# retab-dev/k-LLMs

Measured on NVIDIA H100. Metric: consensus records/sec at n=16 (1M x 32-field); achieved HBM GB/s vs peak, higher is better.
Workload: dtype i32 codes / f64 values

## Files before the change

k_llms_b200/csrc/kc_numeric.cuh:

```cuda
#pragma once

#include <type_traits>
#include <utility>

#include "kc_common.cuh"
#include "kc_csa.cuh"
#include "kc_vote.cuh"

namespace kc {

constexpr uint32_t kNoneHi = (uint32_t)(KC_F64_NONE_BITS >> 32);
constexpr uint32_t kAbsentHi = (uint32_t)(KC_F64_ABSENT_BITS >> 32);
constexpr uint32_t kKeyNonFinite = 0xFFE00000u;

__device__ __forceinline__ int ffs_m(uint32_t m) { return __ffs((int)m); }
__device__ __forceinline__ int ffs_m(uint64_t m) { return __ffsll((long long)m); }
__device__ __forceinline__ int clz_m(uint32_t m) { return __clz((int)m); }
__device__ __forceinline__ int clz_m(uint64_t m) { return __clzll((long long)m); }

__device__ __constant__ double kPow10[13] = {1e-6, 1e-5, 1e-4, 1e-3, 1e-2, 1e-1, 1.0, 1e1, 1e2, 1e3, 1e4, 1e5, 1e6};


__device__ __forceinline__ double lds_f64(uint32_t addr) {
    double v;
    asm volatile("ld.shared.f64 %0, [%1];" : "=d"(v) : "r"(addr));
    return v;
}
__device__ __forceinline__ void sts_f64(uint32_t addr, double v) {
    asm volatile("st.shared.f64 [%0], %1;" ::"r"(addr), "d"(v) : "memory");
}
__device__ __forceinline__ uint2 lds_u32x2(uint32_t addr) {
    uint2 v;
    asm volatile("ld.shared.v2.u32 {%0,%1}, [%2];" : "=r"(v.x), "=r"(v.y) : "r"(addr));
    return v;
}

struct PlaneRow {
    uint32_t base, pitch;
    __device__ __forceinline__ uint32_t addr(uint32_t elem) const { return base + elem * pitch; }
    __device__ __forceinline__ uint32_t addr_mad(uint32_t elem) const {
        uint32_t a;
        asm("mad.lo.u32 %0, %1, %2, %3;" : "=r"(a) : "r"(elem), "r"(pitch), "r"(base));
        return a;
    }
};


template <typename F>
__device__ __forceinline__ double np_sum(F f, int n) {
    double res;
    if (n < 8) {
        res = -0.0;
        for (int i = 0; i < n; ++i) res = __dadd_rn(res, f(i));
    } else {
        double r0 = f(0), r1 = f(1), r2 = f(2), r3 = f(3), r4 = f(4), r5 = f(5), r6 = f(6), r7 = f(7);
        int i = 8;
        const int n8 = n - (n & 7);
        for (; i < n8; i += 8) {
            r0 = __dadd_rn(r0, f(i + 0));
            r1 = __dadd_rn(r1, f(i + 1));
            r2 = __dadd_rn(r2, f(i + 2));
            r3 = __dadd_rn(r3, f(i + 3));
            r4 = __dadd_rn(r4, f(i + 4));
            r5 = __dadd_rn(r5, f(i + 5));
            r6 = __dadd_rn(r6, f(i + 6));
            r7 = __dadd_rn(r7, f(i + 7));
        }
        res = __dadd_rn(__dadd_rn(__dadd_rn(r0, r1), __dadd_rn(r2, r3)), __dadd_rn(__dadd_rn(r4, r5), __dadd_rn(r6, r7)));
        for (; i < n; ++i) res = __dadd_rn(res, f(i));
    }
    return __dadd_rn(0.0, res);
}

template <typename Row>
__device__ __forceinline__ double np_mean(const Row &xs, int s, int len) {
    return __ddiv_rn(np_sum([&](int i) { return lds_f64(xs.addr(s + i)); }, len), (double)len);
}

template <typename Row>
__device__ __forceinline__ double np_mean16(const Row &xs, int s, int len) {
    const uint32_t a0 = xs.addr_mad((uint32_t)s);
    const uint32_t pitch = xs.addr(1) - xs.addr(0);
    double res;
    if (len < 8) {
        res = -0.0;
#pragma unroll
        for (int j = 0; j < 7; ++j)
            if (j < len) res = __dadd_rn(res, lds_f64(a0 + j * pitch));
    } else {
        double r[8];
#pragma unroll
        for (int j = 0; j < 8; ++j) r[j] = lds_f64(a0 + j * pitch);
        int tail = 8;
        if (len >= 16) {
#pragma unroll
            for (int j = 0; j < 8; ++j) r[j] = __dadd_rn(r[j], lds_f64(a0 + (8 + j) * pitch));
            tail = 16;
        }
        res = __dadd_rn(__dadd_rn(__dadd_rn(r[0], r[1]), __dadd_rn(r[2], r[3])),
                        __dadd_rn(__dadd_rn(r[4], r[5]), __dadd_rn(r[6], r[7])));
#pragma unroll
        for (int j = 0; j < 7; ++j)
            if (tail + j < len) res = __dadd_rn(res, lds_f64(a0 + (tail + j) * pitch));
    }
    return __ddiv_rn(__dadd_rn(0.0, res), (double)len);
}

template <typename Row>
__device__ __forceinline__ double np_median(const Row &xs, int s, int len) {
    if (len & 1) return __dadd_rn(0.0, __dadd_rn(-0.0, lds_f64(xs.addr(s + len / 2))));
    return __ddiv_rn(
        __dadd_rn(0.0, __dadd_rn(__dadd_rn(-0.0, lds_f64(xs.addr(s + len / 2 - 1))), lds_f64(xs.addr(s + len / 2)))), 2.0);
}

template <typename Row>
__device__ __forceinline__ double np_std(const Row &xs, int s, int len) {
    const double mean = np_mean(xs, s, len);
    const double ss = np_sum(
        [&](int i) {
            const double d = __dadd_rn(lds_f64(xs.addr(s + i)), -mean);
            return __dmul_rn(d, d);
        },
        len);
    return __dsqrt_rn(__ddiv_rn(ss, (double)len));
}

__device__ __forceinline__ double dmax(double a, double b) { return a > b ? a : b; }

__device__ __forceinline__ bool is_close(double a, double b, double rel_eps, double abs_eps) {
    const double denom = dmax(dmax(fabs(a), fabs(b)), 1.0);
    return fabs(__dadd_rn(a, -b)) <= dmax(abs_eps, __dmul_rn(rel_eps, denom));
}

__device__ __forceinline__ bool is_close_pow10(double a, double b, double rel_eps, double abs_eps) {
    if (a == 0.0 || b == 0.0) return is_close(a, b, rel_eps, abs_eps);
    for (int k = 0; k < 13; ++k)
        if (is_close(a, __dmul_rn(b, kPow10[k]), rel_eps, abs_eps)) return true;
    return false;
}

struct TieResult {
    double value;
    int support;
};

template <typename M, typename Row>
__device__ __noinline__ TieResult numeric_tie(const Row xs, M starts, int m, int top, double rel_eps, double abs_eps) {
    int best_s = -1, best_support = 0;
    double best_spread = 0.0, best_center = 0.0;
    M sk = starts;
    while (sk) {
        const int s = ffs_m(sk) - 1;
        sk &= sk - 1;
        const int e = sk ? ffs_m(sk) - 1 : m;
        const int len = e - s;
        if (len != top) continue;
        const double center = np_median(xs, s, len);
        int support = top;
        M so = starts;
        while (so) {
            const int os = ffs_m(so) - 1;
            so &= so - 1;
            const int oe = so ? ffs_m(so) - 1 : m;
            const int olen = oe - os;
            if (olen >= top) continue;
            const double oc = np_median(xs, os, olen);
            if (is_close(center, oc, rel_eps, abs_eps) || is_close(fabs(center), fabs(oc), rel_eps, abs_eps) ||
                is_close_pow10(center, oc, rel_eps, abs_eps))
                support += olen;
        }
        const double spread = len > 1 ? np_std(xs, s, len) : 0.0;
        const bool better = best_s < 0 || support > best_support ||
                            (support == best_support &&
                             (spread < best_spread || (spread == best_spread && fabs(center) > fabs(best_center))));
        if (better) {
            best_s = s;
            best_support = support;
            best_spread = spread;
            best_center = center;
        }
    }
    return TieResult{np_mean(xs, best_s, top), best_support};
}


template <int N>
struct BatcherNet {
    int a[N * N / 2 + 1];
    int b[N * N / 2 + 1];
    int count;
    constexpr BatcherNet() : a{}, b{}, count(0) {
        for (int p = 1; p < N; p *= 2)
            for (int k = p; k >= 1; k /= 2)
                for (int j = k % p; j <= N - 1 - k; j += 2 * k)
                    for (int i = 0; i < k; ++i)
                        if (i + j + k < N && (i + j) / (2 * p) == (i + j + k) / (2 * p)) {
                            a[count] = i + j;
                            b[count] = i + j + k;
                            ++count;
                        }
    }
};

template <int A, int B, int N>
__device__ __forceinline__ void compare_exchange(uint32_t (&x)[N]) {
    const uint32_t lo = min(x[A], x[B]), hi = max(x[A], x[B]);
    x[A] = lo;
    x[B] = hi;
}

template <int N, size_t... I>
__device__ __forceinline__ void sort_keys_impl(uint32_t (&x)[N], std::index_sequence<I...>) {
    constexpr BatcherNet<N> net{};
    (compare_exchange<net.a[I], net.b[I], N>(x), ...);
}

template <int N>
__device__ __forceinline__ void sort_keys(uint32_t (&x)[N]) {
    constexpr BatcherNet<N> net{};
    sort_keys_impl<N>(x, std::make_index_sequence<net.count>{});
}

__device__ __forceinline__ uint32_t far_bit(double d, double p, double q, double thr, uint32_t bit) {
    uint32_t r;
    asm("{\n\t"
        ".reg .pred c;\n\t"
        "setp.le.f64 c, %1, %2;\n\t"
        "setp.le.or.f64 c, %1, %3, c;\n\t"
        "setp.le.or.f64 c, %1, %4, c;\n\t"
        "selp.u32 %0, 0, %5, c;\n\t"
        "}"
        : "=r"(r)
        : "d"(d), "d"(p), "d"(q), "d"(thr), "r"(bit));
    return r;
}

template <typename Row>
__device__ __noinline__ void repair_sorted_prefix(const Row row, int m) {
    for (int i = 1; i < m; ++i) {
        const double v = lds_f64(row.addr(i));
        int j = i - 1;
        while (j >= 0) {
            const double u = lds_f64(row.addr(j));
            if (!(u > v)) break;
            sts_f64(row.addr(j + 1), u);
            --j;
        }
        sts_f64(row.addr(j + 1), v);
    }
}


template <int N, typename Row>
__device__ __forceinline__ void numeric_core(const uint32_t (&hi)[N], const Row row, double rel_eps, double abs_eps,
                                             double thr, double &value, uint32_t &meta) {
    using M = typename MaskOf<N>::type;
    static_assert(N >= 2 && (N & (N - 1)) == 0, "N must be a power of two >= 2");
    constexpr uint32_t IDX = N - 1;
    const double qnan = __longlong_as_double(0x7FF8000000000000LL);

    constexpr uint32_t Z_NONE = ((kNoneHi ^ 0x80000000u) - 0x00100000u) - kKeyNonFinite;
    static_assert(kAbsentHi == kNoneHi + 1, "tags must be adjacent high words");
    uint32_t key[N];
    uint32_t census = 0;
#pragma unroll
    for (int i = 0; i < N; ++i) {
        const uint32_t s = (uint32_t)((int32_t)hi[i] >> 31);
        const uint32_t t = (hi[i] ^ (s | 0x80000000u)) - 0x00100000u;
        key[i] = (t | IDX) - (IDX - (uint32_t)i);
        const uint32_t z = t - kKeyNonFinite;
        const uint32_t u = z - Z_NONE;
        const uint32_t tagged_inc = (u < 2u) ? (u + 0x10100u) : 0x100u;
        census += (z < 0x00200000u) ? tagged_inc : 0u;
    }
    const int m = N - (int)((census >> 8) & 0xFFu);
    const int present = N - (int)(census & 0xFFu);
    const int nn = N - (int)(census >> 16);
    if (nn == 0) {
        value = qnan;
        meta = pack_meta(0, 0, 0, present, 0);
        return;
    }
    if (nn == 1) {
        int idx = 0;
        for (int i = 0; i < N; ++i) {
            const uint32_t h = lds_u32x2(row.addr(i)).y;
            if (h != kNoneHi && h != kAbsentHi) idx = i;
        }
        value = lds_f64(row.addr(idx));
        meta = pack_meta(idx, 1, 1, present, KC_FLAG_HAS_VALUE | KC_FLAG_SINGLE);
        return;
    }
    if (m == 0) {
        value = qnan;
        meta = pack_meta(0, 0, nn, present, KC_FLAG_NO_FINITE);
        return;
    }

    sort_keys<N>(key);
    double xs[N];
#pragma unroll
    for (int k = 0; k < N; ++k) xs[k] = lds_f64(row.addr_mad(key[k] & IDX));

    bool unsorted = false;
#pragma unroll
    for (int k = 1; k < N; ++k) unsorted |= xs[k] < xs[k - 1];
#pragma unroll
    for (int k = 0; k < N; ++k) sts_f64(row.addr(k), xs[k]);
    if (unsorted) {
        repair_sorted_prefix<Row>(row, m);
#pragma unroll
        for (int k = 0; k < N; ++k) xs[k] = lds_f64(row.addr(k));
    }

    M starts = 1;
    {
        double p_prev = __dmul_rn(rel_eps, xs[0]);
#pragma unroll
        for (int k = 1; k < N; ++k) {
            const double p = __dmul_rn(rel_eps, xs[k]);
            const double d = __dadd_rn(xs[k], -xs[k - 1]);
            starts |= (M)far_bit(d, p, -p_prev, thr, 1u << (k & 31)) << (k & 32);
            p_prev = p;
        }
    }
    if (m < N) starts &= (M(1) << m) - 1;

    int top = 0, n_top = 0, top_s = 0;
    {
        const int c = m >> 1;
        const M below = starts & ((M(2) << c) - 1);
        const int s0 = (int)(sizeof(M) * 8 - 1) - clz_m(below);
        const M above = c + 1 < (int)(sizeof(M) * 8) ? (starts >> (c + 1)) : M(0);
        const int e0 = above ? c + ffs_m(above) : m;
        if (2 * (e0 - s0) > m) {
            top = e0 - s0;
            n_top = 1;
            top_s = s0;
        }
    }
    if (n_top == 0) {
        M sk = starts;
        while (sk) {
            const int s = ffs_m(sk) - 1;
            sk &= sk - 1;
            const int e = sk ? ffs_m(sk) - 1 : m;
            const int len = e - s;
            if (len > top) {
                top = len;
                n_top = 1;
                top_s = s;
            } else if (len == top) {
                ++n_top;
            }
        }
    }
    uint32_t flags = KC_FLAG_HAS_VALUE;
    int support = top;
    if (n_top == 1) {
        if constexpr (N <= 16 && std::is_same<Row, PlaneRow>::value)
            value = np_mean16(row, top_s, top);
        else
            value = np_mean(row, top_s, top);
    } else {
        const TieResult tr = numeric_tie<M, Row>(row, starts, m, top, rel_eps, abs_eps);
        value = tr.value;
        support = tr.support;
        flags |= KC_FLAG_TIE;
    }
    meta = pack_meta(0, support, nn, present, flags);
}

__device__ __forceinline__ void numeric_pair(uint2 a, uint2 b, double rel_eps, double abs_eps, double &value, uint32_t &meta) {
    const bool a_abs = a.y == kAbsentHi, b_abs = b.y == kAbsentHi;
    const bool a_nn = !a_abs && a.y != kNoneHi, b_nn = !b_abs && b.y != kNoneHi;
    const bool a_fin = a_nn && (a.y & 0x7FF00000u) != 0x7FF00000u, b_fin = b_nn && (b.y & 0x7FF00000u) != 0x7FF00000u;
    const uint32_t present = (a_abs ? 0u : 1u) + (b_abs ? 0u : 1u), nn = (a_nn ? 1u : 0u) + (b_nn ? 1u : 0u);
    const double va = __hiloint2double((int)a.y, (int)a.x), vb = __hiloint2double((int)b.y, (int)b.x);
    const double qnan = __longlong_as_double(0x7FF8000000000000ll);
    if (nn == 0) {
        value = qnan;
        meta = pack_meta(0, 0, 0, present, 0);
    } else if (nn == 1) {
        value = a_nn ? va : vb;
        meta = pack_meta(a_nn ? 0u : 1u, 1, 1, present, KC_FLAG_HAS_VALUE | KC_FLAG_SINGLE);
    } else if (!a_fin && !b_fin) {
        value = qnan;
        meta = pack_meta(0, 0, 2, present, KC_FLAG_NO_FINITE);
    } else if (a_fin != b_fin) {
        value = __dadd_rn(0.0, __dadd_rn(-0.0, a_fin ? va : vb));
        meta = pack_meta(0, 1, 2, present, KC_FLAG_HAS_VALUE);
    } else {
        const bool swap = va > vb;
        const double lo = swap ? vb : va, hi = swap ? va : vb;
        if (is_close(lo, hi, rel_eps, abs_eps)) {
            value = __ddiv_rn(__dadd_rn(0.0, __dadd_rn(__dadd_rn(-0.0, lo), hi)), 2.0);
            meta = pack_meta(0, 2, 2, present, KC_FLAG_HAS_VALUE);
        } else {
            const double c_lo = __dadd_rn(0.0, __dadd_rn(-0.0, lo)), c_hi = __dadd_rn(0.0, __dadd_rn(-0.0, hi));
            value = fabs(c_hi) > fabs(c_lo) ? c_hi : c_lo;
            meta = pack_meta(0, 1, 2, present, KC_FLAG_HAS_VALUE | KC_FLAG_TIE);
        }
    }
}

__global__ void __launch_bounds__(256) numeric_pairs_kernel(const double *__restrict__ vals, int64_t n_units, double rel_eps, double abs_eps,
                                                            double *__restrict__ out_value, uint32_t *__restrict__ out_meta) {
    const int64_t stride = (int64_t)gridDim.x * blockDim.x;
    int64_t u = (int64_t)blockIdx.x * blockDim.x + threadIdx.x;
    int4 cur[4];
    if (u < n_units) {
        const int4 *p = reinterpret_cast<const int4 *>(vals) + u * 4;
#pragma unroll
        for (int q = 0; q < 4; ++q) cur[q] = ldg_nc_v4(p + q);
    }
    for (; u < n_units; u += stride) {
        int4 nxt[4];
        if (u + stride < n_units) {
            const int4 *p = reinterpret_cast<const int4 *>(vals) + (u + stride) * 4;
#pragma unroll
            for (int q = 0; q < 4; ++q) nxt[q] = ldg_nc_v4(p + q);
        }
        double v[4];
        uint32_t m[4];
#pragma unroll
        for (int q = 0; q < 4; ++q)
            numeric_pair(make_uint2((uint32_t)cur[q].x, (uint32_t)cur[q].y), make_uint2((uint32_t)cur[q].z, (uint32_t)cur[q].w), rel_eps, abs_eps,
                         v[q], m[q]);
        double *ov = out_value + u * 4;
        asm volatile("st.global.L1::no_allocate.v2.f64 [%0], {%1,%2};" ::"l"(ov), "d"(v[0]), "d"(v[1]) : "memory");
        asm volatile("st.global.L1::no_allocate.v2.f64 [%0], {%1,%2};" ::"l"(ov + 2), "d"(v[2]), "d"(v[3]) : "memory");
        asm volatile("st.global.L1::no_allocate.v4.u32 [%0], {%1,%2,%3,%4};" ::"l"(out_meta + u * 4), "r"(m[0]), "r"(m[1]), "r"(m[2]), "r"(m[3])
                     : "memory");
#pragma unroll
        for (int q = 0; q < 4; ++q) cur[q] = nxt[q];
    }
}

__device__ __forceinline__ void cex(double &a, double &b) {
    const bool sw = a > b;
    const double lo = sw ? b : a, hi = sw ? a : b;
    a = lo;
    b = hi;
}

__device__ __forceinline__ void numeric_quad(const uint2 (&w)[4], double rel_eps, double abs_eps, double &value, uint32_t &meta) {
    const double pinf = __longlong_as_double(0x7FF0000000000000ll), qnan = __longlong_as_double(0x7FF8000000000000ll);
    uint32_t present = 0, nn = 0, m = 0, first_nn = 0;
    double x[4];
#pragma unroll
    for (int i = 3; i >= 0; --i) {
        const bool absent = w[i].y == kAbsentHi, none = w[i].y == kNoneHi, fin = (w[i].y & 0x7FF00000u) != 0x7FF00000u;
        present += absent ? 0u : 1u;
        const bool is_nn = !absent && !none;
        nn += is_nn ? 1u : 0u;
        first_nn = is_nn ? (uint32_t)i : first_nn;
        m += fin ? 1u : 0u;
        x[i] = fin ? __hiloint2double((int)w[i].y, (int)w[i].x) : pinf;
    }
    if (nn == 0) {
        value = qnan;
        meta = pack_meta(0, 0, 0, present, 0);
        return;
    }
    if (nn == 1) {
        const uint2 c = first_nn == 0 ? w[0] : (first_nn == 1 ? w[1] : (first_nn == 2 ? w[2] : w[3]));
        value = __hiloint2double((int)c.y, (int)c.x);
        meta = pack_meta(first_nn, 1, 1, present, KC_FLAG_HAS_VALUE | KC_FLAG_SINGLE);
        return;
    }
    if (m == 0) {
        value = qnan;
        meta = pack_meta(0, 0, nn, present, KC_FLAG_NO_FINITE);
        return;
    }
    cex(x[0], x[1]);
    cex(x[2], x[3]);
    cex(x[0], x[2]);
    cex(x[1], x[3]);
    cex(x[1], x[2]);
    const bool b0 = m > 1 && is_close(x[0], x[1], rel_eps, abs_eps);
    const bool b1 = m > 2 && is_close(x[1], x[2], rel_eps, abs_eps);
    const bool b2 = m > 3 && is_close(x[2], x[3], rel_eps, abs_eps);
    uint32_t best_len = 0, best_start = 0, n_top = 0, cur_len = 0, cur_start = 0;
#pragma unroll
    for (int i = 0; i < 4; ++i) {
        const bool in = (uint32_t)i < m;
        const bool joins = i > 0 && (i == 1 ? b0 : (i == 2 ? b1 : b2));
        cur_start = joins ? cur_start : (uint32_t)i;
        cur_len = joins ? cur_len + 1u : 1u;
        const bool ends = in && ((uint32_t)i + 1u == m || !(i == 0 ? b0 : (i == 1 ? b1 : b2)));
        if (ends) {
            if (cur_len > best_len) {
                best_len = cur_len;
                best_start = cur_start;
                n_top = 1;
            } else if (cur_len == best_len) {
                ++n_top;
            }
        }
    }
    auto mean_of = [&](uint32_t s, uint32_t z) -> double {
        double acc = -0.0;
#pragma unroll
        for (int i = 0; i < 4; ++i)
            if ((uint32_t)i >= s && (uint32_t)i < s + z) acc = __dadd_rn(acc, x[i]);
        return __ddiv_rn(__dadd_rn(0.0, acc), (double)z);
    };
    if (n_top == 1) {
        value = mean_of(best_start, best_len);
        meta = pack_meta(0, best_len, nn, present, KC_FLAG_HAS_VALUE);
        return;
    }
    if (best_len == 1) {
        double best = __dadd_rn(0.0, __dadd_rn(-0.0, x[0]));
#pragma unroll
        for (int i = 1; i < 4; ++i) {
            const double c = __dadd_rn(0.0, __dadd_rn(-0.0, x[i]));
            if ((uint32_t)i < m && fabs(c) > fabs(best)) best = c;
        }
        value = best;
        meta = pack_meta(0, 1, nn, present, KC_FLAG_HAS_VALUE | KC_FLAG_TIE);
        return;
    }
    auto pair_stats = [&](double a, double b, double &mean, double &sd) {
        mean = __ddiv_rn(__dadd_rn(0.0, __dadd_rn(__dadd_rn(-0.0, a), b)), 2.0);
        const double ta = __dadd_rn(a, -mean), tb = __dadd_rn(b, -mean);
        const double ss = __dadd_rn(0.0, __dadd_rn(__dadd_rn(-0.0, __dmul_rn(ta, ta)), __dmul_rn(tb, tb)));
        sd = __dsqrt_rn(__ddiv_rn(ss, 2.0));
    };
    double ma, sa, mb, sb;
    pair_stats(x[0], x[1], ma, sa);
    pair_stats(x[2], x[3], mb, sb);
    const bool second = sb < sa || (sb == sa && fabs(mb) > fabs(ma));
    value = second ? mb : ma;
    meta = pack_meta(0, 2, nn, present, KC_FLAG_HAS_VALUE | KC_FLAG_TIE);
}

__global__ void __launch_bounds__(256) numeric_quads_kernel(const double *__restrict__ vals, int64_t n_units, double rel_eps, double abs_eps,
                                                            double *__restrict__ out_value, uint32_t *__restrict__ out_meta) {
    const int64_t stride = (int64_t)gridDim.x * blockDim.x;
    int64_t u = (int64_t)blockIdx.x * blockDim.x + threadIdx.x;
    int4 cur[4];
    if (u < n_units) {
        const int4 *p = reinterpret_cast<const int4 *>(vals) + u * 4;
#pragma unroll
        for (int q = 0; q < 4; ++q) cur[q] = ldg_nc_v4(p + q);
    }
    for (; u < n_units; u += stride) {
        int4 nxt[4];
        if (u + stride < n_units) {
            const int4 *p = reinterpret_cast<const int4 *>(vals) + (u + stride) * 4;
#pragma unroll
            for (int q = 0; q < 4; ++q) nxt[q] = ldg_nc_v4(p + q);
        }
        double v[2];
        uint32_t m[2];
#pragma unroll
        for (int g = 0; g < 2; ++g) {
            const uint2 w[4] = {make_uint2((uint32_t)cur[2 * g].x, (uint32_t)cur[2 * g].y), make_uint2((uint32_t)cur[2 * g].z, (uint32_t)cur[2 * g].w),
                                make_uint2((uint32_t)cur[2 * g + 1].x, (uint32_t)cur[2 * g + 1].y),
                                make_uint2((uint32_t)cur[2 * g + 1].z, (uint32_t)cur[2 * g + 1].w)};
            numeric_quad(w, rel_eps, abs_eps, v[g], m[g]);
        }
        asm volatile("st.global.L1::no_allocate.v2.f64 [%0], {%1,%2};" ::"l"(out_value + u * 2), "d"(v[0]), "d"(v[1]) : "memory");
        asm volatile("st.global.L1::no_allocate.v2.u32 [%0], {%1,%2};" ::"l"(out_meta + u * 2), "r"(m[0]), "r"(m[1]) : "memory");
#pragma unroll
        for (int q = 0; q < 4; ++q) cur[q] = nxt[q];
    }
}



template <int NP, int T, bool PREFETCH>
__global__ void __launch_bounds__(T) numeric_direct_kernel(const double *__restrict__ vals, int64_t n_groups, int n,
                                                           double rel_eps, double abs_eps, double *__restrict__ out_value,
                                                           uint32_t *__restrict__ out_meta, const __grid_constant__ OutRoute mc) {
    extern __shared__ __align__(1024) uint8_t smem_raw[];
    const PlaneRow row{smem_u32(smem_raw) + threadIdx.x * 8u, T * 8u};
    const double thr = abs_eps > rel_eps ? abs_eps : rel_eps;
    const int64_t stride = (int64_t)gridDim.x * T;
    int64_t g = (int64_t)blockIdx.x * T + threadIdx.x;
    int4 cur[NP / 2 > 0 ? NP / 2 : 1];
    if constexpr (PREFETCH) {
        if (g < n_groups) {
            const int4 *p4 = reinterpret_cast<const int4 *>(vals + g * NP);
#pragma unroll
            for (int q = 0; q < NP / 2; ++q) cur[q] = ldg_nc_v4(p4 + q);
        }
    }
    for (; g < n_groups; g += stride) {
        uint32_t hi[NP];
        if constexpr (PREFETCH) {
            int4 nxt[NP / 2];
            if (g + stride < n_groups) {
                const int4 *p4 = reinterpret_cast<const int4 *>(vals + (g + stride) * NP);
#pragma unroll
                for (int q = 0; q < NP / 2; ++q) nxt[q] = ldg_nc_v4(p4 + q);
            }
#pragma unroll
            for (int q = 0; q < NP / 2; ++q) {
                hi[2 * q + 0] = (uint32_t)cur[q].y;
                hi[2 * q + 1] = (uint32_t)cur[q].w;
                sts_f64(row.addr(2 * q + 0), __hiloint2double(cur[q].y, cur[q].x));
                sts_f64(row.addr(2 * q + 1), __hiloint2double(cur[q].w, cur[q].z));
            }
            double v;
            uint32_t m;
            numeric_core<NP, PlaneRow>(hi, row, rel_eps, abs_eps, thr, v, m);
            store_out_f64(out_value + g, v, mc);
            store_out_u32(out_meta + g, m, mc);
#pragma unroll
            for (int q = 0; q < NP / 2; ++q) cur[q] = nxt[q];
        } else {
            const double *p = vals + g * n;
            if (n == NP) {
                const int4 *p4 = reinterpret_cast<const int4 *>(p);
#pragma unroll
                for (int q = 0; q < NP / 2; ++q) {
                    const int4 t = ldg_nc_v4(p4 + q);
                    hi[2 * q + 0] = (uint32_t)t.y;
                    hi[2 * q + 1] = (uint32_t)t.w;
                    sts_f64(row.addr(2 * q + 0), __hiloint2double(t.y, t.x));
                    sts_f64(row.addr(2 * q + 1), __hiloint2double(t.w, t.z));
                }
            } else {
#pragma unroll
                for (int i = 0; i < NP; ++i) {
                    const double v = (i < n) ? __ldg(p + i) : __longlong_as_double((long long)KC_F64_ABSENT_BITS);
                    hi[i] = (uint32_t)__double2hiint(v);
                    sts_f64(row.addr(i), v);
                }
            }
            double v;
            uint32_t m;
            numeric_core<NP, PlaneRow>(hi, row, rel_eps, abs_eps, thr, v, m);
            store_out_f64(out_value + g, v, mc);
            store_out_u32(out_meta + g, m, mc);
        }
    }
}


__device__ __forceinline__ void count_equal(uint32_t x, uint32_t key, uint32_t &n) {
    asm("{\n\t.reg .pred p;\n\t"
        "setp.eq.u32 p, %1, %2;\n\t"
        "@p add.u32 %0, %0, 1;\n\t}"
        : "+r"(n)
        : "r"(x), "r"(key));
}

__device__ __forceinline__ void match_cell(uint32_t h, uint32_t l, uint32_t hv, uint32_t lv, uint32_t &c, uint32_t &bad) {
    asm("{\n\t.reg .pred p;\n\t"
        "setp.eq.u32 p, %2, %4;\n\t"
        "@p add.u32 %0, %0, 1;\n\t"
        "@p lop3.b32 %1, %1, %3, %5, 0xF6;\n\t}"
        : "+r"(c), "+r"(bad)
        : "r"(h), "r"(l), "r"(hv), "r"(lv));
}

constexpr uint32_t kFastBias = 0x00100000u;

struct FastDecision {
    double v;
    uint32_t c, tagged, absent;
};

template <int N>
__device__ __forceinline__ bool numeric_fast_decide(const uint32_t (&x)[N], const uint32_t (&lo)[N], uint32_t top, double rel_eps,
                                                    double thr, FastDecision &out) {
    constexpr uint32_t X_NONE = kNoneHi + kFastBias, X_ABSENT = kAbsentHi + kFastBias;
    constexpr int PLANES = 32 - __builtin_clz((unsigned)N);
    uint32_t plane[PLANES];
    bit_counts(x, plane);
    const uint32_t xv = plane[PLANES - 1] | plane[PLANES - 2], lv = at_least_half(lo);
    uint32_t nonfinite = 0;
#pragma unroll
    for (int k = 0; k < PLANES; ++k) nonfinite += (plane[k] >> 31) << k;
    uint32_t c = 0, bad = 0, below = 0, above = 0xFFFFFFFFu, low_nf = 0xFFFFFFFFu, absent = 0;
    const uint32_t neg_xv = 0u - xv, neg_xv1 = ~xv;
#pragma unroll
    for (int i = 0; i < N; ++i) {
        below = max(below, x[i] + neg_xv);
        above = min(above, x[i] + neg_xv1);
        low_nf = min(low_nf, x[i] + 0x80000000u);
        match_cell(x[i], lo[i], xv, lv, c, bad);
    }
    if (top == kAbsentHi) {
#pragma unroll
        for (int i = 0; i < N; ++i) count_equal(x[i], X_ABSENT, absent);
    }
    const uint32_t tagged = nonfinite;
    if (top > kAbsentHi || (xv & 0x80000000u) != 0 || bad != 0 || 2 * c + nonfinite <= (uint32_t)N || tagged > (uint32_t)(N - 2) ||
        (nonfinite != 0 && low_nf < X_NONE - 0x80000000u))
        return false;
    const uint32_t hv = xv - kFastBias;
    const double v = __hiloint2double((int)hv, (int)lv);
    const uint32_t hb = hv + below, ha = hv + above + 1u;
    const double db = __dadd_rn(v, -__hiloint2double((int)hb, -1));
    const double da = __dadd_rn(__hiloint2double((int)ha, 0), -v);
    const bool far_b = db > thr && db > __dmul_rn(rel_eps, v);
    const bool far_a = da > thr && da > __dmul_rn(rel_eps, __hiloint2double((int)ha, -1));
    const bool has_b = below >= 0x80000000u, has_a = above < 0x7FFFFFFFu && ha < 0x7FF00000u;
    if ((has_b && !far_b) || (has_a && !far_a)) return false;
    out.v = v;
    out.c = c;
    out.tagged = tagged;
    out.absent = absent;
    return true;
}

template <int N>
__device__ __forceinline__ void numeric_fast_finish(const FastDecision &d, double &value, uint32_t &meta) {
    const double v = d.v;
    const uint32_t c = d.c, tagged = d.tagged, absent = d.absent;
    double res = -0.0;
    if (c >= 8) {
        double r = v;
#pragma unroll
        for (int k = 2; k <= N / 8; ++k)
            if ((int)(c >> 3) >= k) r = __dadd_rn(r, v);
        res = __dmul_rn(r, 8.0);
    }
    const uint32_t tail = c & 7u;
#pragma unroll
    for (int k = 1; k <= 7; ++k)
        if ((int)tail >= k) res = __dadd_rn(res, v);
    value = __ddiv_rn(__dadd_rn(0.0, res), (double)c);
    meta = (c << 6) + (((uint32_t)N - tagged) << 13) + (((uint32_t)N - absent) << 20) + ((uint32_t)KC_FLAG_HAS_VALUE << 27);
}

template <int NP, int T>
__global__ void __launch_bounds__(T) numeric_direct_fast_kernel(const double *__restrict__ vals, int64_t n_groups, double rel_eps,
                                                                double abs_eps, double *__restrict__ out_value,
                                                                uint32_t *__restrict__ out_meta, const __grid_constant__ OutRoute ) {
    extern __shared__ __align__(1024) uint8_t smem_raw[];
    __shared__ int64_t defer_q[T / 32][64];
    const PlaneRow row{smem_u32(smem_raw) + threadIdx.x * 8u, T * 8u};
    const double thr = abs_eps > rel_eps ? abs_eps : rel_eps;
    const int lane = threadIdx.x & 31;
    int64_t *my_q = defer_q[threadIdx.x >> 5];
    int q_count = 0;
    const int64_t stride = (int64_t)gridDim.x * T;
    const int64_t g0 = (int64_t)blockIdx.x * T + threadIdx.x;

    const uint32_t warp_plane = smem_u32(smem_raw) + (threadIdx.x & ~31u) * 8u;
    auto drain = [&](int count) {
        if (lane < count) {
            const int64_t g = my_q[lane];
            uint32_t hi[NP];
#pragma unroll
            for (int i = 0; i < NP; ++i) hi[i] = lds_u32x2(row.addr(i)).y;
            double v;
            uint32_t m;
            numeric_core<NP, PlaneRow>(hi, row, rel_eps, abs_eps, thr, v, m);
            store_local_f64(out_value + g, v);
            store_local_u32(out_meta + g, m);
        }
        __syncwarp();
    };

    int4 cur[NP / 2];
    if (g0 < n_groups) {
        const int4 *p4 = reinterpret_cast<const int4 *>(vals + g0 * NP);
#pragma unroll
        for (int q = 0; q < NP / 2; ++q) cur[q] = ldg_nc_v4(p4 + q);
    }
    for (int64_t gw = g0 - lane; gw < n_groups; gw += stride) {
        const int64_t g = gw + lane;
        int4 nxt[NP / 2];
        if (g + stride < n_groups) {
            const int4 *p4 = reinterpret_cast<const int4 *>(vals + (g + stride) * NP);
#pragma unroll
            for (int q = 0; q < NP / 2; ++q) nxt[q] = ldg_nc_v4(p4 + q);
        }
        uint32_t x[NP], lo[NP], top = 0;
#pragma unroll
        for (int q = 0; q < NP / 2; ++q) {
            lo[2 * q + 0] = (uint32_t)cur[q].x;
            x[2 * q + 0] = (uint32_t)cur[q].y + kFastBias;
            lo[2 * q + 1] = (uint32_t)cur[q].z;
            x[2 * q + 1] = (uint32_t)cur[q].w + kFastBias;
            top = max(top, max((uint32_t)cur[q].y, (uint32_t)cur[q].w));
        }
        FastDecision fd;
        const bool decided = numeric_fast_decide<NP>(x, lo, top, rel_eps, thr, fd);
        const bool defer = !decided && g < n_groups;
        const uint32_t dm = __ballot_sync(0xFFFFFFFFu, defer);
        if (defer) {
            const uint32_t slot = (uint32_t)q_count + (uint32_t)__popc(dm & ((1u << lane) - 1u));
            my_q[slot] = g;
            if (slot < 32u) {
#pragma unroll
                for (int i = 0; i < NP; ++i)
                    sts_f64(warp_plane + slot * 8u + (uint32_t)i * (T * 8u), __hiloint2double((int)(x[i] - kFastBias), (int)lo[i]));
            }
        }
        q_count += __popc(dm);
        if (decided && g < n_groups) {
            double v;
            uint32_t m;
            numeric_fast_finish<NP>(fd, v, m);
            store_local_f64(out_value + g, v);
            store_local_u32(out_meta + g, m);
        }
        __syncwarp();
        if (q_count >= 32) {
            drain(32);
            q_count -= 32;
            const int64_t moved = (lane < q_count) ? my_q[32 + lane] : 0;
            __syncwarp();
            if (lane < q_count) {
                my_q[lane] = moved;
                const int4 *p4 = reinterpret_cast<const int4 *>(vals + moved * NP);
#pragma unroll
                for (int q = 0; q < NP / 2; ++q) {
                    const int4 v4 = ldg_nc_v4(p4 + q);
                    sts_f64(row.addr(2 * q + 0), __hiloint2double(v4.y, v4.x));
                    sts_f64(row.addr(2 * q + 1), __hiloint2double(v4.w, v4.z));
                }
            }
            __syncwarp();
        }
#pragma unroll
        for (int q = 0; q < NP / 2; ++q) cur[q] = nxt[q];
    }
    if (q_count > 0) drain(q_count);
}

template <int N, int WARPS, int STAGES, int MIN_CTAS>
__global__ void __launch_bounds__(WARPS * 32, MIN_CTAS) numeric_tma_fast_kernel(const __grid_constant__ CUtensorMap tmap,
                                                                      const double *__restrict__ in, int64_t n_groups,
                                                                      double rel_eps, double abs_eps,
                                                                      double *__restrict__ out_value,
                                                                      uint32_t *__restrict__ out_meta, const __grid_constant__ OutRoute ) {
    constexpr int ROW_BYTES = N * 8;
    constexpr int BOX_ROWS_PER_GROUP = ROW_BYTES > 128 ? ROW_BYTES / 128 : 1;
    constexpr uint32_t TILE_BYTES = 32 * ROW_BYTES;
    constexpr int T = WARPS * 32;
    static_assert(TILE_BYTES % 1024 == 0, "warp tile must keep the swizzle atom alignment");
    extern __shared__ __align__(1024) uint8_t smem_raw[];
    uint8_t *smem = reinterpret_cast<uint8_t *>((reinterpret_cast<uintptr_t>(smem_raw) + 1023) & ~uintptr_t(1023));
    __shared__ __align__(8) uint64_t full_bar[WARPS * STAGES];
    __shared__ int64_t defer_q[WARPS][64];

    const int lane = threadIdx.x & 31;
    const int warp = threadIdx.x >> 5;
    uint8_t *my_smem = smem + (size_t)warp * STAGES * TILE_BYTES;
    uint64_t *my_bar = full_bar + warp * STAGES;
    int64_t *my_q = defer_q[warp];
    int q_count = 0;
    const PlaneRow row{smem_u32(smem + (size_t)WARPS * STAGES * TILE_BYTES) + threadIdx.x * 8u, T * 8u};
    const double thr = abs_eps > rel_eps ? abs_eps : rel_eps;

    const int64_t n_tiles = (n_groups + 31) >> 5;
    const int64_t first = (int64_t)blockIdx.x * WARPS + warp;
    const int64_t step = (int64_t)gridDim.x * WARPS;
    uint64_t policy = 0;

    if (lane == 0) {
        tma_prefetch_desc(&tmap);
#pragma unroll
        for (int s = 0; s < STAGES; ++s) mbar_init(&my_bar[s], 1);
        fence_barrier_init();
        policy = policy_evict_normal();
#pragma unroll
        for (int s = 0; s < STAGES; ++s) {
            const int64_t t = first + (int64_t)s * step;
            if (t < n_tiles) {
                mbar_arrive_expect_tx(&my_bar[s], TILE_BYTES);
                tma_load_2d(my_smem + (size_t)s * TILE_BYTES, &tmap, 0, (int32_t)(t * 32 * BOX_ROWS_PER_GROUP), &my_bar[s],
                            policy);
            }
        }
    }
    __syncwarp();

    const uint32_t warp_plane = smem_u32(smem + (size_t)WARPS * STAGES * TILE_BYTES) + (uint32_t)warp * 32u * 8u;
    auto drain = [&](int count) {
        if (lane < count) {
            const int64_t g = my_q[lane];
            uint32_t hi[N];
#pragma unroll
            for (int i = 0; i < N; ++i) hi[i] = lds_u32x2(row.addr(i)).y;
            double v;
            uint32_t m;
            numeric_core<N, PlaneRow>(hi, row, rel_eps, abs_eps, thr, v, m);
            store_local_f64(out_value + g, v);
            store_local_u32(out_meta + g, m);
        }
        __syncwarp();
    };

    int stage = 0;
    uint32_t parity = 0;
    for (int64_t t = first; t < n_tiles; t += step) {
        mbar_wait(&my_bar[stage], parity);
        const uint32_t base = smem_u32(my_smem + (size_t)stage * TILE_BYTES);
        const uint32_t row_off = (uint32_t)lane * ROW_BYTES;
        uint32_t x[N], lo[N];
        uint32_t touch = 0, top = 0;
#pragma unroll
        for (int q = 0; q < N / 2; ++q) {
            const int4 v4 = lds_v4(base + Swizzle<ROW_BYTES>::apply(row_off + q * 16));
            lo[2 * q + 0] = (uint32_t)v4.x;
            x[2 * q + 0] = (uint32_t)v4.y + kFastBias;
            lo[2 * q + 1] = (uint32_t)v4.z;
            x[2 * q + 1] = (uint32_t)v4.w + kFastBias;
            top = max(top, max((uint32_t)v4.y, (uint32_t)v4.w));
            touch |= (uint32_t)v4.w;
        }
        const uint32_t order = __shfl_sync(0xFFFFFFFFu, touch, 0) ^ touch;
        if (lane == 0) {
            const int64_t tn = t + (int64_t)STAGES * step;
            if (tn < n_tiles) {
                mbar_arrive_expect_tx(&my_bar[stage], TILE_BYTES);
                tma_load_2d(my_smem + (size_t)stage * TILE_BYTES, &tmap, 0,
                            (int32_t)(tn * 32 * BOX_ROWS_PER_GROUP) + (int32_t)order, &my_bar[stage], policy);
            }
        }
        const int64_t g = t * 32 + lane;
        FastDecision fd;
        const bool decided = numeric_fast_decide<N>(x, lo, top, rel_eps, thr, fd);
        const bool defer = !decided && g < n_groups;
        const uint32_t dm = __ballot_sync(0xFFFFFFFFu, defer);
        if (defer) {
            const uint32_t slot = (uint32_t)q_count + (uint32_t)__popc(dm & ((1u << lane) - 1u));
            my_q[slot] = g;
            if (slot < 32u) {
#pragma unroll
                for (int i = 0; i < N; ++i)
                    sts_f64(warp_plane + slot * 8u + (uint32_t)i * (T * 8u), __hiloint2double((int)(x[i] - kFastBias), (int)lo[i]));
            }
        }
        q_count += __popc(dm);
        if (decided && g < n_groups) {
            double v;
            uint32_t m;
            numeric_fast_finish<N>(fd, v, m);
            store_local_f64(out_value + g, v);
            store_local_u32(out_meta + g, m);
        }
        __syncwarp();
        if (q_count >= 32) {
            drain(32);
            q_count -= 32;
            const int64_t moved = (lane < q_count) ? my_q[32 + lane] : 0;
            __syncwarp();
            if (lane < q_count) {
                my_q[lane] = moved;
                const int4 *p4 = reinterpret_cast<const int4 *>(in + moved * N);
#pragma unroll
                for (int q = 0; q < N / 2; ++q) {
                    const int4 v4 = ldg_nc_v4(p4 + q);
                    sts_f64(row.addr(2 * q + 0), __hiloint2double(v4.y, v4.x));
                    sts_f64(row.addr(2 * q + 1), __hiloint2double(v4.w, v4.z));
                }
            }
            __syncwarp();
        }
        if (++stage == STAGES) {
            stage = 0;
            parity ^= 1;
        }
    }
    if (q_count > 0) drain(q_count);
}

template <int N, int WARPS, int STAGES, int MIN_CTAS>
__global__ void __launch_bounds__(WARPS * 32, MIN_CTAS) numeric_tma_kernel(const __grid_constant__ CUtensorMap tmap,
                                                                 int64_t n_groups, double rel_eps, double abs_eps,
                                                                 double *__restrict__ out_value,
                                                                 uint32_t *__restrict__ out_meta, const __grid_constant__ OutRoute mc) {
    constexpr int ROW_BYTES = N * 8;
    constexpr int BOX_ROWS_PER_GROUP = ROW_BYTES > 128 ? ROW_BYTES / 128 : 1;
    constexpr uint32_t TILE_BYTES = 32 * ROW_BYTES;
    constexpr int T = WARPS * 32;
    static_assert(TILE_BYTES % 1024 == 0, "warp tile must keep the swizzle atom alignment");
    extern __shared__ __align__(1024) uint8_t smem_raw[];
    uint8_t *smem = reinterpret_cast<uint8_t *>((reinterpret_cast<uintptr_t>(smem_raw) + 1023) & ~uintptr_t(1023));
    __shared__ __align__(8) uint64_t full_bar[WARPS * STAGES];

    const int lane = threadIdx.x & 31;
    const int warp = threadIdx.x >> 5;
    uint8_t *my_smem = smem + (size_t)warp * STAGES * TILE_BYTES;
    uint64_t *my_bar = full_bar + warp * STAGES;
    const PlaneRow row{smem_u32(smem + (size_t)WARPS * STAGES * TILE_BYTES) + threadIdx.x * 8u, T * 8u};
    const double thr = abs_eps > rel_eps ? abs_eps : rel_eps;

    const int64_t n_tiles = (n_groups + 31) >> 5;
    const int64_t first = (int64_t)blockIdx.x * WARPS + warp;
    const int64_t step = (int64_t)gridDim.x * WARPS;
    uint64_t policy = 0;

    if (lane == 0) {
        tma_prefetch_desc(&tmap);
#pragma unroll
        for (int s = 0; s < STAGES; ++s) mbar_init(&my_bar[s], 1);
        fence_barrier_init();
        policy = policy_evict_normal();
#pragma unroll
        for (int s = 0; s < STAGES; ++s) {
            const int64_t t = first + (int64_t)s * step;
            if (t < n_tiles) {
                mbar_arrive_expect_tx(&my_bar[s], TILE_BYTES);
                tma_load_2d(my_smem + (size_t)s * TILE_BYTES, &tmap, 0, (int32_t)(t * 32 * BOX_ROWS_PER_GROUP), &my_bar[s],
                            policy);
            }
        }
    }
    __syncwarp();

    int stage = 0;
    uint32_t parity = 0;
    for (int64_t t = first; t < n_tiles; t += step) {
        mbar_wait(&my_bar[stage], parity);
        const uint32_t base = smem_u32(my_smem + (size_t)stage * TILE_BYTES);
        const uint32_t row_off = (uint32_t)lane * ROW_BYTES;
        uint32_t hi[N];
        uint32_t touch = 0;
#pragma unroll
        for (int q = 0; q < N / 2; ++q) {
            const int4 v4 = lds_v4(base + Swizzle<ROW_BYTES>::apply(row_off + q * 16));
            hi[2 * q + 0] = (uint32_t)v4.y;
            hi[2 * q + 1] = (uint32_t)v4.w;
            sts_f64(row.addr(2 * q + 0), __hiloint2double(v4.y, v4.x));
            sts_f64(row.addr(2 * q + 1), __hiloint2double(v4.w, v4.z));
            touch |= (uint32_t)v4.w;
        }
        const uint32_t order = __shfl_sync(0xFFFFFFFFu, touch, 0) ^ touch;
        if (lane == 0) {
            const int64_t tn = t + (int64_t)STAGES * step;
            if (tn < n_tiles) {
                mbar_arrive_expect_tx(&my_bar[stage], TILE_BYTES);
                tma_load_2d(my_smem + (size_t)stage * TILE_BYTES, &tmap, 0,
                            (int32_t)(tn * 32 * BOX_ROWS_PER_GROUP) + (int32_t)order, &my_bar[stage], policy);
            }
        }
        const int64_t g = t * 32 + lane;
        if (g < n_groups) {
            double v;
            uint32_t m;
            numeric_core<N, PlaneRow>(hi, row, rel_eps, abs_eps, thr, v, m);
            store_out_f64(out_value + g, v, mc);
            store_out_u32(out_meta + g, m, mc);
        }
        if (++stage == STAGES) {
            stage = 0;
            parity ^= 1;
        }
    }
}

}
```

Baseline: 970.8 million.

## Resolve near-cluster extras in fast numeric path instead of deferring to slow path

For N>=16, the fast numeric decision no longer bails out when a neighbouring value lies within epsilon of the majority value. It walks up to two close neighbours on each side, checks they are unique and chain-close, and records them in the decision word. The finish step then reproduces the reference summation order, including those extras, to compute the mean. The goal is to keep more groups off the deferred slow path, at the cost of extra per-group loops and floating-point work plus more register pressure.

```diff
diff --git a/k_llms_b200/csrc/kc_numeric.cuh b/k_llms_b200/csrc/kc_numeric.cuh
--- a/k_llms_b200/csrc/kc_numeric.cuh
+++ b/k_llms_b200/csrc/kc_numeric.cuh
@@ -663,8 +663,18 @@
 
 struct FastDecision {
     double v;
-    uint32_t c, tagged, absent;
+    double e0, e1;
+    uint32_t word;
 };
+
+template <int N>
+constexpr bool kWalkExtras = N >= 16;
+
+__device__ __forceinline__ bool certainly_far(double f, uint32_t h, bool below, double rel_eps, double thr) {
+    const double d = below ? __dadd_rn(f, -__hiloint2double((int)h, -1)) : __dadd_rn(__hiloint2double((int)h, 0), -f);
+    const double mag = below ? f : __hiloint2double((int)h, -1);
+    return d > thr && d > __dmul_rn(rel_eps, mag);
+}
 
 template <int N>
 __device__ __forceinline__ bool numeric_fast_decide(const uint32_t (&x)[N], const uint32_t (&lo)[N], uint32_t top, double rel_eps,
@@ -697,37 +707,106 @@
     const uint32_t hv = xv - kFastBias;
     const double v = __hiloint2double((int)hv, (int)lv);
     const uint32_t hb = hv + below, ha = hv + above + 1u;
-    const double db = __dadd_rn(v, -__hiloint2double((int)hb, -1));
-    const double da = __dadd_rn(__hiloint2double((int)ha, 0), -v);
-    const bool far_b = db > thr && db > __dmul_rn(rel_eps, v);
-    const bool far_a = da > thr && da > __dmul_rn(rel_eps, __hiloint2double((int)ha, -1));
     const bool has_b = below >= 0x80000000u, has_a = above < 0x7FFFFFFFu && ha < 0x7FF00000u;
-    if ((has_b && !far_b) || (has_a && !far_a)) return false;
+    const bool need_b = has_b && !certainly_far(v, hb, true, rel_eps, thr);
+    const bool need_a = has_a && !certainly_far(v, ha, false, rel_eps, thr);
     out.v = v;
-    out.c = c;
-    out.tagged = tagged;
-    out.absent = absent;
+    out.word = (c << 6) + (((uint32_t)N - tagged) << 13) + (((uint32_t)N - absent) << 20) + ((uint32_t)KC_FLAG_HAS_VALUE << 27);
+    out.e0 = out.e1 = v;
+    if constexpr (!kWalkExtras<N>) {
+        if (need_b || need_a) return false;
+    }
+    uint32_t xn = need_b ? hb + kFastBias : 0u, xa = need_a ? ha + kFastBias : 0u;
+    if (xn == 0u) {
+        xn = xa;
+        xa = 0u;
+    }
+    while (xn != 0u) {
+        const uint32_t nb = out.word & 3u, na = (out.word >> 2) & 3u;
+        if (nb + na == 2u) return false;
+        const bool down = xn < xv;
+        const uint32_t sm = down ? 0u : 0xFFFFFFFFu, neg = 0u - (xn ^ sm);
+        uint32_t cnt = 0, ln = 0, beyond = 0;
+#pragma unroll
+        for (int i = 0; i < N; ++i) {
+            beyond = max(beyond, (x[i] ^ sm) + neg);
+            asm("{\n\t.reg .pred p;\n\t"
+                "setp.eq.u32 p, %2, %4;\n\t"
+                "@p add.u32 %0, %0, 1;\n\t"
+                "@p mov.b32 %1, %3;\n\t}"
+                : "+r"(cnt), "+r"(ln)
+                : "r"(x[i]), "r"(lo[i]), "r"(xn));
+        }
+        if (cnt != 1u) return false;
+        const double e = __hiloint2double((int)(xn - kFastBias), (int)ln);
+        const double f = (down ? nb : na) ? out.e0 : v;
+        const double a = down ? e : f, b = down ? f : e;
+        const bool close = far_bit(__dadd_rn(b, -a), __dmul_rn(rel_eps, b), -__dmul_rn(rel_eps, a), thr, 1u) == 0u;
+        bool side_done = !close;
+        if (close) {
+            out.e1 = out.e0;
+            out.e0 = e;
+            out.word += down ? 1u : 4u;
+            const uint32_t hn = (down ? xn + beyond : xn - beyond) - kFastBias;
+            const bool exists = beyond >= 0x80000000u && (down || hn < 0x7FF00000u);
+            side_done = !exists || certainly_far(e, hn, down, rel_eps, thr);
+            xn = hn + kFastBias;
+        }
+        if (side_done) {
+            xn = xa;
+            xa = 0u;
+        }
+    }
     return true;
 }
 
 template <int N>
 __device__ __forceinline__ void numeric_fast_finish(const FastDecision &d, double &value, uint32_t &meta) {
     const double v = d.v;
-    const uint32_t c = d.c, tagged = d.tagged, absent = d.absent;
-    double res = -0.0;
-    if (c >= 8) {
-        double r = v;
-#pragma unroll
-        for (int k = 2; k <= N / 8; ++k)
-            if ((int)(c >> 3) >= k) r = __dadd_rn(r, v);
-        res = __dmul_rn(r, 8.0);
-    }
-    const uint32_t tail = c & 7u;
+    const uint32_t c = (d.word >> 6) & 127u;
+    if constexpr (!kWalkExtras<N>) {
+        double res = -0.0;
+        if (c >= 8) {
+            double r = v;
+#pragma unroll
+            for (int k = 2; k <= N / 8; ++k)
+                if ((int)(c >> 3) >= k) r = __dadd_rn(r, v);
+            res = __dmul_rn(r, 8.0);
+        }
+#pragma unroll
+        for (int k = 1; k <= 7; ++k)
+            if ((int)(c & 7u) >= k) res = __dadd_rn(res, v);
+        value = __ddiv_rn(__dadd_rn(0.0, res), (double)c);
+        meta = d.word;
+        return;
+    }
+    const uint32_t nb = d.word & 3u, na = (d.word >> 2) & 3u;
+    const uint32_t z = c + nb + na, q = z >> 3, t = z & 7u;
+    const double f0 = nb == 0u ? v : (na == 0u ? d.e0 : d.e1), f1 = nb == 2u ? d.e1 : v;
+    const double l2 = na == 2u ? d.e1 : v, l1 = na == 0u ? v : d.e0;
+    double r0 = f0, r1 = f1, rp = -0.0;
+#pragma unroll
+    for (int k = 2; k <= N / 8; ++k)
+        if ((int)q >= k) {
+            r0 = __dadd_rn(r0, v);
+            r1 = __dadd_rn(r1, v);
+            rp = __dadd_rn(rp, v);
+        }
+    const double r6 = __dadd_rn(rp, t == 0u ? l2 : v), r7 = __dadd_rn(rp, t == 0u ? l1 : (t == 1u ? l2 : v));
+    const double r2 = __dadd_rn(rp, v), s23 = __dadd_rn(r2, r2);
+    const double tree = __dadd_rn(__dadd_rn(__dadd_rn(r0, r1), s23), __dadd_rn(s23, __dadd_rn(r6, r7)));
+    const bool small = z < 8u;
+    const uint32_t sb = small ? nb : 0u, sa = small ? na : min(na, t), sv = small ? c : t - sa;
+    double res = small ? -0.0 : tree;
+    if (sb >= 1u) res = __dadd_rn(res, f0);
+    if (sb >= 2u) res = __dadd_rn(res, f1);
 #pragma unroll
     for (int k = 1; k <= 7; ++k)
-        if ((int)tail >= k) res = __dadd_rn(res, v);
-    value = __ddiv_rn(__dadd_rn(0.0, res), (double)c);
-    meta = (c << 6) + (((uint32_t)N - tagged) << 13) + (((uint32_t)N - absent) << 20) + ((uint32_t)KC_FLAG_HAS_VALUE << 27);
+        if ((int)sv >= k) res = __dadd_rn(res, v);
+    if (sa >= 2u) res = __dadd_rn(res, l2);
+    if (sa >= 1u) res = __dadd_rn(res, l1);
+    value = __ddiv_rn(__dadd_rn(0.0, res), (double)z);
+    meta = (d.word & ~15u) + ((nb + na) << 6);
 }
 
 template <int NP, int T>
```

After: 1.004 billion, median of 6. +3.4%, better.
